# Eric-qi/RDO-PTQ

Measured on AMD Instinct MI355X. Metric: calibration images/sec (Cheng2020 W8A8 task-oriented RDO-PTQ, image-iterations over all units), higher is better.
Workload: dtype f32

## Files before the change

rdo-ptq_amd/csrc/fused_tail.hip:

```cpp
#include "rdo_common.h"
#include "gather_body.h"

namespace {

using namespace rdo::gq;
typedef unsigned short u16;
typedef unsigned u32x2 __attribute__((ext_vector_type(2)));

inline unsigned loss_grid(long blocks) {
    const long cap = rdo::tuning(rdo::T_TAIL_GRID);
    return (unsigned)(blocks < 1 ? 1 : (blocks > cap ? cap : blocks));
}

using rdo::grid_for;

__device__ __forceinline__ void block_loss_add(float acc, float scale, float* loss_out, int it, int32_t* pub) {
    if (pub && blockIdx.x == 0 && threadIdx.x == 0) *pub = it;
    acc = rdo::block_sum(acc);
    if (threadIdx.x == 0 && loss_out)
        atomicAdd(loss_out + (long)it * RDO_LOG_SLOTS + (blockIdx.x & (RDO_LOG_SLOTS - 1)), acc * scale);
}

__device__ __forceinline__ void load_h2_oct(const H2In& pl, long M, int C, const Oct& o, f32x4& a, f32x4& b) {
    const long pstride = M * C;
    const long e = ((long)(o.c0 >> 4) * M + o.m) * 16 + (o.c0 & 15);
    const u32x4 h = *reinterpret_cast<const u32x4*>(pl.p + e), l = *reinterpret_cast<const u32x4*>(pl.p + pstride + e);
    using rdo::h2_hi;
    using rdo::h2_lo;
    a = f32x4{(h2_lo(h[0]) + h2_lo(l[0])) * pl.inv, (h2_hi(h[0]) + h2_hi(l[0])) * pl.inv, (h2_lo(h[1]) + h2_lo(l[1])) * pl.inv,
              (h2_hi(h[1]) + h2_hi(l[1])) * pl.inv};
    b = f32x4{(h2_lo(h[2]) + h2_lo(l[2])) * pl.inv, (h2_hi(h[2]) + h2_hi(l[2])) * pl.inv, (h2_lo(h[3]) + h2_lo(l[3])) * pl.inv,
              (h2_hi(h[3]) + h2_hi(l[3])) * pl.inv};
}

__global__ __launch_bounds__(256) void gather_qdrop_h2_kernel(Gather g, const int32_t* iter_ptr, int32_t* iter_publish) {
    const int it = *iter_ptr;
// ... 79 lines not shown
            if (res) r[k] = ldq(res + e);
            acc += loss_act_quad(ldq(pre + e), ldq(yrow + e), has_r ? &r[k] : nullptr, act, slope, gs, o[k], g[k], d[k]);
        }
#pragma unroll
        for (int k = 0; k < 2; ++k) {
            if (out) stq(out + e0 + k * Q2, o[k]);
            if (gout) stq(gout + e0 + k * Q2, g[k]);
            if (dpre) stq(dpre + e0 + k * Q2, d[k]);
        }
        if (dpre_planes.p) store_h2_oct(dpre_planes, M, C, oc, d[0], d[1], bad);
    }
    if (dpre_planes.p) rdo::h2_report(bad, dpre_planes.ovf);
    block_loss_add(acc, inv_npix * coef, loss_out, it, iter_pub);
}

__device__ __forceinline__ float loss_gdn_quad(const f32x4& xv, const f32x4& nv, const f32x4& y, const f32x4* r, int inverse, float gs,
                                               f32x4& o, f32x4& g, f32x4& tv) {
    f32x4 rs;
#pragma unroll
    for (int k = 0; k < 4; ++k) {
        rs[k] = __frsqrt_rn(nv[k]);
        o[k] = xv[k] * (inverse ? __fsqrt_rn(nv[k]) : rs[k]);
    }
    if (r) o += *r;
    const f32x4 dd = o - y;
    g = dd * gs;
#pragma unroll
    for (int k = 0; k < 4; ++k)
        tv[k] = inverse ? (0.5f * g[k] * xv[k]) * rs[k] : (-0.5f * g[k] * xv[k]) * (rs[k] * rs[k] * rs[k]);
    return (dd[0] * dd[0] + dd[1] * dd[1]) + (dd[2] * dd[2] + dd[3] * dd[3]);
}

__global__ __launch_bounds__(256) void loss_gdn_bwd_kernel(const float* x, const float* nrm, const float* res, const float* tgt,
                                                           const int32_t* idx_table, const int32_t* iter_ptr, int B, long per_image,
                                                           float inv_npix, float coef, int inverse, float* out, float* gout, float* tbuf,
                                                           float* loss_out, int32_t* iter_pub) {
    const int it = *iter_ptr;
    const long quads = per_image / 4;
    const long total = (long)B * quads;
    const float gs = coef * 2.f * inv_npix;
    float acc = 0.f;
    for (long q = (long)blockIdx.x * blockDim.x + threadIdx.x; q < total; q += (long)gridDim.x * blockDim.x) {
        const int b = (int)(q / quads);
        const long off = (q - (long)b * quads) * 4;
        const long e = (long)b * per_image + off;
        f32x4 r, o, g, tv;
        if (res) r = ldq(res + e);
// ... 31 lines not shown
            if (res) r = ldq(res + e);
            acc += loss_gdn_quad(ldq(x + e), ldq(nrm + e), ldq(yrow + e), res ? &r : nullptr, inverse, gs, o[k], g[k], tv[k]);
        }
#pragma unroll
        for (int k = 0; k < 2; ++k) {
            if (out) stq(out + e0 + k * Q2, o[k]);
            stq(gout + e0 + k * Q2, g[k]);
            if (tbuf) stq(tbuf + e0 + k * Q2, tv[k]);
        }
        store_h2_oct(t_planes, M, C, oc, tv[0], tv[1], bad);
    }
    rdo::h2_report(bad, t_planes.ovf);
    block_loss_add(acc, inv_npix * coef, loss_out, it, iter_pub);
}

__device__ __forceinline__ f32x4 gdn_dx_quad(const f32x4& gv, const f32x4& xv, const f32x4& nv, const f32x4& av, int inverse) {
    f32x4 o;
#pragma unroll
    for (int k = 0; k < 4; ++k) {
        const float f = inverse ? __fsqrt_rn(nv[k]) : __frsqrt_rn(nv[k]);
        o[k] = gv[k] * f + 2.f * xv[k] * av[k];
    }
    return o;
}

__global__ __launch_bounds__(256) void gdn_bwd_dx_kernel(const float* g, const float* x, const float* nrm, const float* acc, long n4,
                                                         int inverse, float* dx) {
    for (long q = (long)blockIdx.x * blockDim.x + threadIdx.x; q < n4; q += (long)gridDim.x * blockDim.x) {
        const long e = q * 4;
        stq(dx + e, gdn_dx_quad(ldq(g + e), ldq(x + e), ldq(nrm + e), ldq(acc + e), inverse));
    }
}

__global__ __launch_bounds__(256) void gdn_bwd_dx_pix_kernel(const float* g, const float* x, const float* nrm, const float* acc, long M,
                                                             int C, int inverse, float* dx, H2Out dx_planes) {
    int bad = 0;
    const int ngroups = (C + 31) / 32;
    const long nvb = ((M + 63) / 64) * ngroups;
    for (long vb = blockIdx.x; vb < nvb; vb += gridDim.x) {
        Oct oc;
// ... 269 lines not shown
```

rdo-ptq_amd/csrc/linear_h2.hip:

```cpp
#include <cstdlib>

#include "rdo_common.h"

namespace {

typedef float f32x4 __attribute__((ext_vector_type(4)));
typedef _Float16 f16x8 __attribute__((ext_vector_type(8)));
typedef _Float16 f16x4 __attribute__((ext_vector_type(4)));
typedef unsigned u32x4 __attribute__((ext_vector_type(4)));

constexpr int BM = 64;
constexpr int KB = 192;
constexpr int NC = 192;
constexpr int SLICES = KB / 16;
constexpr int PLANE = SLICES * BM * 32;
constexpr int LDS_BYTES = 2 * PLANE + 2 * BM * 4;

struct LinArgs {
    const float* x;
    const unsigned short* wp;
    const float* bias;
    float* out;
    int M, K, N;
    float inv_wscale;
    int square;
#ifdef RDO_DIAG
    int diag;
#endif
    int epi;
    float* pre;
    const float* aux;
};

__device__ __forceinline__ float pow2f(int e) { return __builtin_bit_cast(float, (unsigned)(e + 127) << 23); }

template <int EPI, bool PART = false>
__global__ __launch_bounds__(256, 3) void linear_h2_kernel(LinArgs a) {
    extern __shared__ __attribute__((aligned(16))) char smem[];
    float* scl = reinterpret_cast<float*>(smem + 2 * PLANE);
    const int tid = threadIdx.x, lane = tid & 63, wave = tid >> 6;
    const int l16 = lane & 15, kg = lane >> 4;
    const int nkb = PART ? (a.K + KB - 1) / KB : a.K / KB, nchunks = PART ? (a.N + NC - 1) / NC : a.N / NC, nblk = a.N / 16, ksteps = a.K / 32;
    const int kvalid4 = PART ? (a.K < KB ? a.K : KB) >> 2 : KB / 4;
    const int nks = PART ? (ksteps < KB / 32 ? ksteps : KB / 32) : KB / 32;
    const bool wave_live = !PART || a.N >= NC || wave * 48 < a.N;
    int wg_tile, wg_chunk;
    {
        const int ntiles = a.M / BM;
        const int id = blockIdx.x, xcd = id & 7, slot = id >> 3;
// ... 27 lines not shown
#pragma unroll
                for (int k = 0; k < 3; ++k)
                    if (l16 + 16 * k >= kvalid4) v[pass][k] = f32x4{0.f, 0.f, 0.f, 0.f};
        }
        if (a.square) {
#pragma unroll
            for (int pass = 0; pass < BM / 16; ++pass)
#pragma unroll
                for (int k = 0; k < 3; ++k) v[pass][k] *= v[pass][k];
        }
#pragma unroll
        for (int pass = 0; pass < BM / 16; ++pass) {
            const int r = pass * 16 + row_in_pass;
            float amax = 0.f;
#pragma unroll
            for (int k = 0; k < 3; ++k)
                amax = fmaxf(amax, fmaxf(fmaxf(fabsf(v[pass][k][0]), fabsf(v[pass][k][1])), fmaxf(fabsf(v[pass][k][2]), fabsf(v[pass][k][3]))));
            amax = fmaxf(amax, __shfl_xor(amax, 8, 16));
            amax = fmaxf(amax, __shfl_xor(amax, 4, 16));
            amax = fmaxf(amax, __shfl_xor(amax, 2, 16));
            amax = fmaxf(amax, __shfl_xor(amax, 1, 16));
            const int e = (int)((__builtin_bit_cast(unsigned, amax) >> 23) & 0xFF) - 127;
            const bool plain = e < -100 || e > 100;
            const float s = plain ? 1.f : pow2f(7 - e);
            if (l16 == 0) scl[(kb & 1) * BM + r] = plain ? 1.f : pow2f(e - 7);
#pragma unroll
            for (int k = 0; k < 3; ++k) {
                const int c4 = l16 + 16 * k;
                const f32x4 xs = v[pass][k] * s;
                const f16x4 hi = __builtin_convertvector(xs, f16x4);
                const f16x4 lo = __builtin_convertvector(xs - __builtin_convertvector(hi, f32x4), f16x4);
                char* dst = smem + (c4 >> 2) * (BM * 32) + r * 32 + (c4 & 3) * 8;
                *reinterpret_cast<f16x4*>(dst) = hi;
                *reinterpret_cast<f16x4*>(dst + PLANE) = lo;
            }
        }
    };

    const u32x4* wbase = reinterpret_cast<const u32x4*>(a.wp) + lane;
    auto load_w = [&](f16x8 (&fw)[2][3], int ks, int chunk) {
        const long b0 = wave_live ? (long)chunk * (NC / 16) + wave * 3 : 0;
#pragma unroll
        for (int p = 0; p < 2; ++p)
#pragma unroll
            for (int i = 0; i < 3; ++i)
                fw[p][i] = __builtin_bit_cast(f16x8, wbase[(((long)p * ksteps + ks) * nblk + b0 + i) * 64]);
    };
    const int fx_lane = (kg >> 1) * (BM * 32) + l16 * 32 + (kg & 1) * 16;
    auto read_x = [&](f16x8 (&fx)[2][4], int ksl) {
// ... 124 lines not shown
        for (int pass = 0; pass < 2; ++pass)
#pragma unroll
            for (int k = 0; k < 3; ++k) asm volatile("" : "+v"(v[pass][k]));
    };
    auto stash = [&](int p) {
        char* buf = smem + (p & 1) * BUF;
#pragma unroll
        for (int pass = 0; pass < 2; ++pass) {
            const int r = pass * 32 + row_in_pass;
            if (a.square) {
#pragma unroll
                for (int k = 0; k < 3; ++k) v[pass][k] *= v[pass][k];
            }
            float amax = 0.f;
#pragma unroll
            for (int k = 0; k < 3; ++k)
                amax = fmaxf(amax, fmaxf(fmaxf(fabsf(v[pass][k][0]), fabsf(v[pass][k][1])), fmaxf(fabsf(v[pass][k][2]), fabsf(v[pass][k][3]))));
            amax = fmaxf(amax, __shfl_xor(amax, 8, 16));
            amax = fmaxf(amax, __shfl_xor(amax, 4, 16));
            amax = fmaxf(amax, __shfl_xor(amax, 2, 16));
            amax = fmaxf(amax, __shfl_xor(amax, 1, 16));
            const int e = (int)((__builtin_bit_cast(unsigned, amax) >> 23) & 0xFF) - 127;
            const bool plain = e < -100 || e > 100;
            const float sc = plain ? 1.f : pow2f(7 - e);
            if (l16 == 0) scl[(p & 3) * BM + r] = plain ? 1.f : pow2f(e - 7);
#pragma unroll
            for (int k = 0; k < 3; ++k) {
                const int c4 = l16 + 16 * k;
                const f32x4 xs = v[pass][k] * sc;
                const f16x4 hi = __builtin_convertvector(xs, f16x4);
                const f16x4 lo = __builtin_convertvector(xs - __builtin_convertvector(hi, f32x4), f16x4);
                char* dst = buf + (c4 >> 2) * (BM * 32) + r * 32 + (c4 & 3) * 8;
                *reinterpret_cast<f16x4*>(dst) = hi;
                *reinterpret_cast<f16x4*>(dst + PLANE) = lo;
            }
        }
    };

    int tl = grp;
    fetch(first + tl, 0);
    if (tid < NCW) bsm[tid] = a.bias ? a.bias[chunk * NCW + tid] : 0.f;
    f16x8 fw[2][KS][NT];
    {
        const u32x4* wbase = reinterpret_cast<const u32x4*>(a.wp) + lane;
        const long b0 = (long)chunk * (NCW / 16) + cg * NT;
        u32x4 raw[2][KS][NT];
#pragma unroll
        for (int p = 0; p < 2; ++p)
#pragma unroll
// ... 239 lines not shown
```

rdo-ptq_amd/hipops/_lib.py:

```python
import ctypes as C
import os

_HERE = os.path.dirname(os.path.abspath(__file__))
LIB_PATH = os.path.join(os.path.dirname(_HERE), "lib", "librdoptq_hip.so")

EPI_NONE, EPI_LRELU, EPI_LRELU_BWD, EPI_GDN, EPI_IGDN, EPI_RELU, EPI_RELU_BWD, EPI_GELU, EPI_GELU_BWD = range(9)
LOG_SLOTS = 32


class ConvDesc(C.Structure):
    _fields_ = [(n, C.c_int32) for n in ("B", "H", "W", "Cin", "Ho", "Wo", "Cout", "KH", "KW", "stride", "pad", "epilogue",
                                         "square_input", "add_residual")]


class AdaDesc(C.Structure):
    _fields_ = [("numel", C.c_int64), ("rows", C.c_int32), ("n_levels", C.c_int32), ("reparam", C.c_int32),
                ("reparam_bound", C.c_float), ("reparam_pedestal", C.c_float), ("KH", C.c_int32), ("KW", C.c_int32),
                ("Cin", C.c_int32)]


class AdaStepItem(C.Structure):
    _fields_ = [("d", AdaDesc), ("w", C.c_void_p), ("delta", C.c_void_p), ("zp", C.c_void_p), ("slabs", C.c_void_p),
                ("nsplit", C.c_int32), ("alpha", C.c_void_p), ("adam_m", C.c_void_p), ("adam_v", C.c_void_p), ("wq", C.c_void_p),
                ("wd", C.c_void_p), ("wq_planes", C.c_void_p), ("wd_planes", C.c_void_p), ("dalpha", C.c_void_p),
# ... 132 lines not shown
    "rdo_pixel_shuffle_h2": (C.c_int, [P, C.c_int32, C.c_int32, C.c_int32, C.c_int32, P, P, C.c_float, P]),
    "rdo_pixel_unshuffle2": (C.c_int, [P, C.c_int32, C.c_int32, C.c_int32, C.c_int32, P, P, C.c_float, P]),
    "rdo_plan_create": (P, []),
    "rdo_plan_destroy": (None, [P]),
    "rdo_plan_begin_record": (C.c_int, [P]),
    "rdo_plan_end_record": (C.c_int, [P]),
    "rdo_plan_suspend_record": (C.c_int, [C.c_int]),
    "rdo_plan_num_ops": (C.c_int, [P]),
    "rdo_plan_run": (C.c_int, [P, C.c_int, C.c_int, P]),
    "rdo_plan_prepare": (C.c_int, [P, C.c_int]),
    "rdo_plan_run_then": (C.c_int, [P, P, C.c_int, P]),
    "rdo_plan_op_info": (C.c_int, [P, C.c_int, C.POINTER(C.c_char_p), C.POINTER(C.c_double), C.POINTER(C.c_double)]),
    "rdo_plan_profile": (C.c_int, [P, C.POINTER(C.c_float), P]),
}
EXPORTS = tuple(_SIGS)

_lib = None


def lib():
    global _lib
    if _lib is None:
        if not os.path.exists(LIB_PATH):
            raise RuntimeError(f"{LIB_PATH} not found: build it with `python __graft_entry__.py` or "
                               f"`make -C rdo-ptq_amd/csrc` (no CPU fallback exists)")
        import torch
        h = C.CDLL(LIB_PATH)
        for name, (res, args) in _SIGS.items():
            fn = getattr(h, name)
            fn.restype, fn.argtypes = res, args
        _lib = h
    return _lib


def check(rc, what=""):
    if rc != 0:
        raise RuntimeError(f"librdoptq_hip {what} failed ({rc}): {lib().rdo_last_error().decode()}")
```

rdo-ptq_amd/hipops/ops.py:

```python
import ctypes as C
import math
import threading

import torch

from . import _lib as L


class H2:
    __slots__ = ("t", "scale", "flag")

    def __init__(self, t, scale, flag=None):
        self.t, self.scale = t, float(scale)
        self.flag = flag
        m, e = math.frexp(self.scale)
        if not (self.scale > 0 and m == 0.5):
            raise ValueError(f"H2 scale must be a positive power of two, got {scale}")

    @property
    def device(self):
        return self.t.device


def _ptr(t):
# ... 1247 lines not shown

def loss_gdn_bwd(x, norm, residual, tgt_cache, idx_table, iter_ptr, coef, inverse, loss_log, grad_out, t=None, t_planes=None, out=None):
    B, per_image = x.shape[0], x[0].numel()
    _bind_out(t_planes)
    L.check(L.lib().rdo_loss_gdn_bwd(_ptr(x), _ptr(norm), _ptr(residual), _ptr(tgt_cache), _ptr(idx_table), _ptr(iter_ptr), B, per_image,
                                     x.shape[-1], coef, int(inverse), _ptr(out), _ptr(grad_out), _ptr(t), _ptr(t_planes), _oscale(t_planes),
                                     _ptr(loss_log), _stream()), "rdo_loss_gdn_bwd")


def gdn_bwd_dx_h2(g, x, norm, acc, inverse, dx=None, dx_planes=None):
    _bind_out(dx_planes)
    L.check(L.lib().rdo_gdn_bwd_dx_h2(_ptr(g), _ptr(x), _ptr(norm), _ptr(acc), g.numel(), g.shape[-1], int(inverse), _ptr(dx),
                                      _ptr(dx_planes), _oscale(dx_planes), _stream()), "rdo_gdn_bwd_dx_h2")


def pixel_shuffle_h2(x, out=None, out_planes=None):
    B, H, W, CC = x.shape
    _bind_out(out_planes)
    L.check(L.lib().rdo_pixel_shuffle_h2(_ptr(x), B, H, W, CC // 4, _ptr(out), _ptr(out_planes), _oscale(out_planes), _stream()),
            "rdo_pixel_shuffle_h2")


def pixel_unshuffle2(x, out=None, out_planes=None):
    B, Hr, Wr, Cc = x.shape
    if out is None and out_planes is None:
        out = torch.empty((B, Hr // 2, Wr // 2, 4 * Cc), device=x.device, dtype=torch.float32)
    _bind_out(out_planes)
    L.check(L.lib().rdo_pixel_unshuffle2(_ptr(x), B, Hr // 2, Wr // 2, Cc, _ptr(out), _ptr(out_planes), _oscale(out_planes), _stream()),
            "rdo_pixel_unshuffle2")
    return out
# ... 20 lines not shown
```

rdo-ptq_amd/quantization/engine.py:

```python
import math
import os
from collections import OrderedDict

import torch

from hipops import _lib as L
from hipops import ops
from hipops.plan import Plan

from . import dp
from .quant_layer import QuantModule
from .quantizer import AdaRoundQuantizer, from_rows, to_rows

UNIT_KINDS = ("layer", "rb", "rbws", "rbu", "rstb")


class DpStallError(RuntimeError):
    """The captured data-parallel loop stopped making progress (`UnitEngine._hb_wait`): a collective inside the graph hangs."""


class IdxStream:
    _spec = None

    @classmethod
# ... 203 lines not shown
        self.task_p = float(task_p)
        self.weight, self.input_prob, self.seed = float(weight), float(input_prob), int(seed) & 0xFFFFFFFF
        self.include_act = include_act_func
        self.use_graph = use_graph
        self.batch_offset = int(batch_offset)
        self.dp_overlap = None if dp_overlap is None else bool(dp_overlap)
        if os.environ.get("RDO_USE_H2") is not None:
            use_h2 = os.environ["RDO_USE_H2"] != "0"
        self.use_h2 = bool(use_h2)
        self.P = {}
        self.batch_step = bool(batch_step)
        self.fuse_splitk = os.environ.get("RDO_FUSE_SPLITK", "1") != "0"
        self.fuse_h2_tail = os.environ.get("RDO_H2_TAIL", "1") != "0"
        self.fold_iter = os.environ.get("RDO_FOLD_ITER", "1") != "0"
        self.fold_gather = os.environ.get("RDO_GATHER_IN_STEP", "1") != "0"
        self._next_gather = None
        self.rd = rd
        if rd is not None:
            metric = rd.get("metric", "mse")
            if metric not in ("mse", "ms-ssim"):
                raise ValueError(f"loss_mode='rd': unknown metric {metric!r} ('mse' or 'ms-ssim')")
            if metric == "ms-ssim" and min(rd["cali"].shape[-2:]) <= 160:
                raise ValueError(f"loss_mode='rd' with metric 'ms-ssim' needs calibration crops with both sides above 160 pixels (five "
                                 f"scales of an 11-tap window); got {tuple(rd['cali'].shape[-2:])}")
            if not include_act_func:
                raise NotImplementedError("calibration engine: loss_mode='rd' substitutes the unit's module OUTPUT (after its fused "
                                          "activation); include_act_func=False optimises the pre-activation and cannot be combined with it")
            fuse_tail = use_h2 = False
            self.use_h2 = False
        self.fuse_tail = bool(fuse_tail)
# ... 117 lines not shown
            else:
                Ho, Wo = self._out_hw(op, H, W)
            t["y"] = self._buf(B, Ho, Wo, op.rows)
            t["dy"] = self._buf(B, Ho, Wo, op.rows)
            t["dpre"] = self._buf(B, Ho, Wo, op.rows)
        elif self.kind == "rb":
            C = o["conv1"].rows
            for n_ in ("h1", "pre2", "out", "dout", "dpre2", "dh1"):
                t[n_] = self._buf(B, H, W, C)
            if "skip" in o:
                t["sk"] = self._buf(B, H, W, C)
        elif self.kind == "rbws":
            c1 = o["conv1"]
            Ho, Wo = self._out_hw(c1, H, W)
            C = c1.rows
            for n_ in ("h1", "c2", "norm", "out", "dout", "t", "acc", "dc2", "dh1"):
                t[n_] = self._buf(B, Ho, Wo, C)
            if "skip" in o:
                t["sk"] = self._buf(B, Ho, Wo, C)
        elif self.kind == "rbu":
            sp = o["subpel_conv"]
            C4 = sp.rows
            r = int(self.mods["upscale"])
            C = C4 // (r * r)
            t["sp"] = self._buf(B, H, W, C4)
            t["h1"] = self._buf(B, H * r, W * r, C)
            t["up"] = self._buf(B, H, W, C4)
            t["ups"] = self._buf(B, H * r, W * r, C)
            for n_ in ("c", "norm", "out", "dout", "t", "acc", "dc", "dh1"):
                t[n_] = self._buf(B, H * r, W * r, C)
            t["dsp"] = self._buf(B, H, W, C4)
            t["dup"] = self._buf(B, H, W, C4)
            self.r = r
        self.t = t
        for op in self.ops.values():
            op.slabs = None

    def _slabs(self, op, x_shape):
        ns = ops.wgrad_nsplit(tuple(x_shape), op.w4, op.stride, op.pad)
        op.slabs = self._buf(ns, *op.w4)
        return op.slabs

    lin_conv = os.environ.get("RDO_CONV1X1_LIN_H2", "1") != "0"

    def _lin_conv_ok(self, op, x):
        if not (self.lin_conv and not self._probing and op.qm.kind == "conv" and op.K == 1 and op.stride == 1 and op.pad == 0 and op.tconv is None):
            return False
        C = x.shape[-1]
        rows = math.prod(x.shape[:-1])
        return rows >= self.LIN_GDN_MIN_ROWS and ops.linear_h2_supported(rows, C, op.w4[0])

# ... 339 lines not shown
            if side_first:
                self._shuffle(t["up"], r, t["ups"])
            self._conv(cv, h1, c)
            if not side_first:
                self._conv(side, x, t["up"])
                self._shuffle(t["up"], r, t["ups"])
            res = t["ups"]
        else:
            self._conv(first, x, h1, epilogue=L.EPI_LRELU)
            if side is not None and side_first:
                self._conv(side, x.f32, t["sk"])
            self._conv(cv, h1, c)
            if side is not None and not side_first:
                self._conv(side, x.f32, t["sk"])
            res = x if side is None else t["sk"]
        if self.fused:
            self._gdn_pool(g, c, t["norm"])
            self._tail_gdn(c, t["norm"], res, rbu, t["dout"], tt)
        else:
            self._conv(g, c, t["out"], epilogue=L.EPI_IGDN if rbu else L.EPI_GDN, aux=c, residual=res, pre=t["norm"], square=True)
            self._loss(t["out"], t["dout"])
        if rbu:
            dup = self._act("dup")
            self._unshuffle(t["dout"], r, dup)
            self._wgrad(side, x, dup)
        elif side is not None:
            self._wgrad(side, x.f32, t["dout"])
        if not self.fused:
            ops.gdn_bwd_t(t["dout"], c, t["norm"], rbu, tt.f32)
        self._gdn_acc(g, tt, t["acc"])
        if dc.planes is not None or c.numel() % 4 == 0:
            ops.gdn_bwd_dx_h2(t["dout"], c, t["norm"], t["acc"], rbu, dx=dc.f32, dx_planes=dc.planes)
        else:
            ops.gdn_bwd_dx(t["dout"], c, t["norm"], t["acc"], rbu, dc.f32)
        self._wgrad(g, c, tt.f32, square=True)
        self._wgrad(cv, h1, dc)
        dh1 = self._act("dh1")
        self._dgrad(cv, dc, dh1, epilogue=L.EPI_LRELU_BWD, aux=h1)
        if rbu:
            dsp = self._act("dsp")
            self._unshuffle(dh1, r, dsp)
            self._split_point()
            self._wgrad(first, x, dsp)
        else:
            self._split_point()
            self._wgrad(first, x, dh1)

    def _probe_amax(self, names):
        saved = ops.set_tuning("conv_x6", 0)
# ... 11 lines not shown
            if op.tc_phase is not None:
                op.expand_phase()

    def _probe_scales(self):
        plan = self._plan_h2()
        if plan is None:
            return
        names = [self.PLANES_AS.get(n, n) for n, f in self._forms(plan, widest=True).items() if f & PLANES]
        amax = self._probe_amax(names)
        self._set_weights(soft=False)
        try:
            amax = torch.maximum(amax, self._probe_amax(names))
        finally:
            self._set_weights(soft=True)
        self._clear_probe()
        if self.world > 1:
            a = amax.to(self.dev)
            a = torch.where(torch.isfinite(a), a, torch.full_like(a, float("inf")))
            torch.distributed.all_reduce(a, op=torch.distributed.ReduceOp.MAX, group=self.group)
            amax = a.cpu()
        if not torch.isfinite(amax).all():
            raise RuntimeError("calibration engine: non-finite activations in the probe iteration")
        if bool((amax <= 0).any()):
            import logging
            logging.getLogger("rdo_ptq.engine").warning(
                "unit with an all-zero tensor in both probe iterations (%s): no fp16 plane scale can be derived, running it on fp32 activations",
                [n for n, a in zip(names, amax) if float(a) <= 0])
            self.use_h2 = False
            return
        self._amax = {n: float(a) for n, a in zip(names, amax)}
# ... 568 lines not shown
```

Baseline: 20440.

## Fuse GDN forward, loss, backward-t and dx into one MFMA kernel

Adds a single kernel that squares the conv output, runs the gamma GEMM on fp16 hi/lo planes with MFMA, applies the GDN/IGDN epilogue with the reconstruction loss, computes t, runs the transposed gamma GEMM and writes dx (optionally as fp16 planes). It replaces the separate pool, tail, gdn_acc and bwd_dx launches and removes the norm/acc intermediate tensors from global memory. The engine uses it when C=192 and the row count is a multiple of 64, and drops the now-unused buffers after probing. The trade-off is a larger, more complex kernel with high register/LDS use and only two blocks per CU, limited to one channel width.

Result: faster. 21240, median of 6 (+3.9%).

```diff
diff --git a/include/rdo_ptq_gdn.h b/include/rdo_ptq_gdn.h
--- /dev/null
+++ b/include/rdo_ptq_gdn.h
@@ -0,0 +1,18 @@
+#ifndef RDO_PTQ_GDN_H
+#define RDO_PTQ_GDN_H
+#include "rdo_ptq_hip.h"
+
+#ifdef __cplusplus
+extern "C" {
+#endif
+
+int rdo_gdn_fwd_bwd_supported(int64_t M, int32_t C);
+int rdo_gdn_fwd_bwd(const float* c, const void* fwd_planes, const void* bwd_planes, float wscale, const float* beta, const float* residual,
+                    const float* tgt_cache, const int32_t* idx_table, const int32_t* iter_ptr, int32_t B, int64_t per_image, int32_t C,
+                    float coef, int32_t inverse, float* out, float* grad_out, float* t, float* dx, void* dx_planes, float dx_scale,
+                    float* loss_out, void* stream);
+
+#ifdef __cplusplus
+}
+#endif
+#endif
diff --git a/rdo-ptq_amd/csrc/fused_tail.hip b/rdo-ptq_amd/csrc/fused_tail.hip
--- a/rdo-ptq_amd/csrc/fused_tail.hip
+++ b/rdo-ptq_amd/csrc/fused_tail.hip
@@ -1,5 +1,6 @@
 #include "rdo_common.h"
 #include "gather_body.h"
+#include "gdn_device.h"
 
 namespace {
 
@@ -13,13 +14,9 @@
 }
 
 using rdo::grid_for;
-
-__device__ __forceinline__ void block_loss_add(float acc, float scale, float* loss_out, int it, int32_t* pub) {
-    if (pub && blockIdx.x == 0 && threadIdx.x == 0) *pub = it;
-    acc = rdo::block_sum(acc);
-    if (threadIdx.x == 0 && loss_out)
-        atomicAdd(loss_out + (long)it * RDO_LOG_SLOTS + (blockIdx.x & (RDO_LOG_SLOTS - 1)), acc * scale);
-}
+using rdo::gdn::block_loss_add;
+using rdo::gdn::loss_gdn_quad;
+using rdo::gdn::gdn_dx_quad;
 
 __device__ __forceinline__ void load_h2_oct(const H2In& pl, long M, int C, const Oct& o, f32x4& a, f32x4& b) {
     const long pstride = M * C;
@@ -129,23 +126,6 @@
     block_loss_add(acc, inv_npix * coef, loss_out, it, iter_pub);
 }
 
-__device__ __forceinline__ float loss_gdn_quad(const f32x4& xv, const f32x4& nv, const f32x4& y, const f32x4* r, int inverse, float gs,
-                                               f32x4& o, f32x4& g, f32x4& tv) {
-    f32x4 rs;
-#pragma unroll
-    for (int k = 0; k < 4; ++k) {
-        rs[k] = __frsqrt_rn(nv[k]);
-        o[k] = xv[k] * (inverse ? __fsqrt_rn(nv[k]) : rs[k]);
-    }
-    if (r) o += *r;
-    const f32x4 dd = o - y;
-    g = dd * gs;
-#pragma unroll
-    for (int k = 0; k < 4; ++k)
-        tv[k] = inverse ? (0.5f * g[k] * xv[k]) * rs[k] : (-0.5f * g[k] * xv[k]) * (rs[k] * rs[k] * rs[k]);
-    return (dd[0] * dd[0] + dd[1] * dd[1]) + (dd[2] * dd[2] + dd[3] * dd[3]);
-}
-
 __global__ __launch_bounds__(256) void loss_gdn_bwd_kernel(const float* x, const float* nrm, const float* res, const float* tgt,
                                                            const int32_t* idx_table, const int32_t* iter_ptr, int B, long per_image,
                                                            float inv_npix, float coef, int inverse, float* out, float* gout, float* tbuf,
@@ -207,16 +187,6 @@
     block_loss_add(acc, inv_npix * coef, loss_out, it, iter_pub);
 }
 
-__device__ __forceinline__ f32x4 gdn_dx_quad(const f32x4& gv, const f32x4& xv, const f32x4& nv, const f32x4& av, int inverse) {
-    f32x4 o;
-#pragma unroll
-    for (int k = 0; k < 4; ++k) {
-        const float f = inverse ? __fsqrt_rn(nv[k]) : __frsqrt_rn(nv[k]);
-        o[k] = gv[k] * f + 2.f * xv[k] * av[k];
-    }
-    return o;
-}
-
 __global__ __launch_bounds__(256) void gdn_bwd_dx_kernel(const float* g, const float* x, const float* nrm, const float* acc, long n4,
                                                          int inverse, float* dx) {
     for (long q = (long)blockIdx.x * blockDim.x + threadIdx.x; q < n4; q += (long)gridDim.x * blockDim.x) {
diff --git a/rdo-ptq_amd/csrc/gdn_device.h b/rdo-ptq_amd/csrc/gdn_device.h
--- /dev/null
+++ b/rdo-ptq_amd/csrc/gdn_device.h
@@ -0,0 +1,87 @@
+#pragma once
+#include "rdo_common.h"
+
+namespace rdo {
+namespace gdn {
+
+typedef float f32x4 __attribute__((ext_vector_type(4)));
+typedef _Float16 f16x4 __attribute__((ext_vector_type(4)));
+
+__device__ __forceinline__ float pow2f(int e) { return __builtin_bit_cast(float, (unsigned)(e + 127) << 23); }
+
+__device__ __forceinline__ float amax_quad(const f32x4& v) { return fmaxf(fmaxf(fabsf(v[0]), fabsf(v[1])), fmaxf(fabsf(v[2]), fabsf(v[3]))); }
+
+__device__ __forceinline__ void token_scale(float amax, float& sc, float& inv) {
+    const int e = (int)((__builtin_bit_cast(unsigned, amax) >> 23) & 0xFF) - 127;
+    const bool plain = e < -100 || e > 100;
+    sc = plain ? 1.f : pow2f(7 - e);
+    inv = plain ? 1.f : pow2f(e - 7);
+}
+
+__device__ __forceinline__ void split_quad_store(const f32x4& v, float sc, char* dst, int plane) {
+    const f32x4 xs = v * sc;
+    const f16x4 hi = __builtin_convertvector(xs, f16x4);
+    const f16x4 lo = __builtin_convertvector(xs - __builtin_convertvector(hi, f32x4), f16x4);
+    *reinterpret_cast<f16x4*>(dst) = hi;
+    *reinterpret_cast<f16x4*>(dst + plane) = lo;
+}
+
+__device__ __forceinline__ void block_loss_add(float acc, float scale, float* loss_out, int it, int32_t* pub) {
+    if (pub && blockIdx.x == 0 && threadIdx.x == 0) *pub = it;
+    acc = rdo::block_sum(acc);
+    if (threadIdx.x == 0 && loss_out)
+        atomicAdd(loss_out + (long)it * RDO_LOG_SLOTS + (blockIdx.x & (RDO_LOG_SLOTS - 1)), acc * scale);
+}
+
+__device__ __forceinline__ void block_loss_add8(float acc, float scale, float* loss_out, int it, int32_t* pub, float* red) {
+    if (pub && blockIdx.x == 0 && threadIdx.x == 0) *pub = it;
+    for (int o = 32; o > 0; o >>= 1) acc += __shfl_down(acc, o, 64);
+    if ((threadIdx.x & 63) == 0) red[threadIdx.x >> 6] = acc;
+    __syncthreads();
+    if (threadIdx.x == 0 && loss_out) {
+        float v = red[0];
+#pragma unroll
+        for (int w = 1; w < 8; ++w) v += red[w];
+        atomicAdd(loss_out + (long)it * RDO_LOG_SLOTS + (blockIdx.x & (RDO_LOG_SLOTS - 1)), v * scale);
+    }
+}
+
+__device__ __forceinline__ float loss_gdn_quad(const f32x4& xv, const f32x4& nv, const f32x4& y, const f32x4* r, int inverse, float gs,
+                                               f32x4& o, f32x4& g, f32x4& tv) {
+    f32x4 rs;
+#pragma unroll
+    for (int k = 0; k < 4; ++k) {
+        rs[k] = __frsqrt_rn(nv[k]);
+        o[k] = xv[k] * (inverse ? __fsqrt_rn(nv[k]) : rs[k]);
+    }
+    if (r) o += *r;
+    const f32x4 dd = o - y;
+    g = dd * gs;
+#pragma unroll
+    for (int k = 0; k < 4; ++k)
+        tv[k] = inverse ? (0.5f * g[k] * xv[k]) * rs[k] : (-0.5f * g[k] * xv[k]) * (rs[k] * rs[k] * rs[k]);
+    return (dd[0] * dd[0] + dd[1] * dd[1]) + (dd[2] * dd[2] + dd[3] * dd[3]);
+}
+
+__device__ __forceinline__ void gdn_dx_pre(const f32x4& gv, const f32x4& xv, const f32x4& nv, int inverse, f32x4& p, f32x4& q) {
+#pragma unroll
+    for (int k = 0; k < 4; ++k) {
+        const float f = inverse ? __fsqrt_rn(nv[k]) : __frsqrt_rn(nv[k]);
+        p[k] = gv[k] * f;
+        q[k] = 2.f * xv[k];
+    }
+}
+__device__ __forceinline__ f32x4 gdn_dx_fin(const f32x4& p, const f32x4& q, const f32x4& av) {
+    f32x4 o;
+#pragma unroll
+    for (int k = 0; k < 4; ++k) o[k] = p[k] + q[k] * av[k];
+    return o;
+}
+__device__ __forceinline__ f32x4 gdn_dx_quad(const f32x4& gv, const f32x4& xv, const f32x4& nv, const f32x4& av, int inverse) {
+    f32x4 p, q;
+    gdn_dx_pre(gv, xv, nv, inverse, p, q);
+    return gdn_dx_fin(p, q, av);
+}
+
+}
+}
diff --git a/rdo-ptq_amd/csrc/gdn_fused.hip b/rdo-ptq_amd/csrc/gdn_fused.hip
--- /dev/null
+++ b/rdo-ptq_amd/csrc/gdn_fused.hip
@@ -0,0 +1,277 @@
+#include "rdo_common.h"
+#include "gather_body.h"
+#include "gdn_device.h"
+#include "../../include/rdo_ptq_gdn.h"
+
+namespace {
+
+using namespace rdo::gdn;
+using rdo::gq::H2Out;
+typedef _Float16 f16x8 __attribute__((ext_vector_type(8)));
+typedef unsigned u32x4 __attribute__((ext_vector_type(4)));
+typedef unsigned u32x2 __attribute__((ext_vector_type(2)));
+typedef unsigned short u16;
+
+constexpr int BM = 64;
+constexpr int CH = 192;
+constexpr int KS = CH / 32;
+constexpr int NBLK = CH / 16;
+constexpr int PLANE = (CH / 16) * BM * 32;
+constexpr int LDS_BYTES = 2 * PLANE + BM * 4 + 4 * BM * 4 + 8 * 4;
+
+struct GdnArgs {
+    const float* c;
+    const u16* wf;
+    const u16* wb;
+    const float* beta;
+    const float* res;
+    const float* tgt;
+    const int32_t* idx;
+    const int32_t* iter;
+    int32_t* pub;
+    int B, ntiles, inverse;
+    long per_image, M;
+    float inv_wscale, inv_npix, coef;
+    float* out;
+    float* gout;
+    float* t;
+    float* dx;
+    H2Out dxp;
+    float* loss_out;
+};
+
+__device__ __forceinline__ const f32x4& ldq(const float* p) { return *reinterpret_cast<const f32x4*>(p); }
+__device__ __forceinline__ void stq(float* p, const f32x4& v) { *reinterpret_cast<f32x4*>(p) = v; }
+
+template <bool INV, bool RES>
+__global__ __launch_bounds__(512, 2) void gdn_fwd_bwd_kernel(GdnArgs a) {
+    extern __shared__ __attribute__((aligned(16))) char smem[];
+    float* scl = reinterpret_cast<float*>(smem + 2 * PLANE);
+    float* wmax = scl + BM;
+    float* wsum = wmax + 4 * BM;
+    const int tid = threadIdx.x, lane = tid & 63, wave = __builtin_amdgcn_readfirstlane(tid >> 6);
+    const int cg = wave & 3, th = wave >> 2;
+    const int l16 = lane & 15, kg = lane >> 4;
+    const int it = *a.iter;
+    const float gs = a.coef * 2.f * a.inv_npix;
+    const long ppi = a.per_image / CH;
+    const int ch0 = 48 * cg + 4 * kg;
+    const unsigned lane_e = (unsigned)((32 * th + l16) * CH + ch0);
+    float lsum = 0.f;
+    int bad = 0;
+
+    const auto rs_f = __builtin_amdgcn_make_buffer_rsrc(const_cast<u16*>(a.wf), 0, 2 * CH * CH * 2, 0x00020000);
+    const auto rs_b = __builtin_amdgcn_make_buffer_rsrc(const_cast<u16*>(a.wb), 0, 2 * CH * CH * 2, 0x00020000);
+    auto load_w = [&](f16x8 (&fw)[2][3], const decltype(rs_f)& planes, int ks) {
+#pragma unroll
+        for (int p = 0; p < 2; ++p)
+#pragma unroll
+            for (int i = 0; i < 3; ++i)
+                fw[p][i] = __builtin_bit_cast(f16x8, __builtin_amdgcn_raw_buffer_load_b128(planes, (unsigned)lane * 16u,
+                                                                                           ((p * KS + ks) * NBLK + cg * 3 + i) * 1024, 0));
+    };
+    const int fx_lane = (kg >> 1) * (BM * 32) + (32 * th + l16) * 32 + (kg & 1) * 16;
+    auto gemm = [&](const decltype(rs_f)& planes, f32x4 (&acc)[3][2]) {
+        f16x8 fw[2][2][3];
+        load_w(fw[0], planes, 0);
+        __syncthreads();
+#pragma unroll
+        for (int i = 0; i < 3; ++i)
+#pragma unroll
+            for (int j = 0; j < 2; ++j) acc[i][j] = f32x4{0.f, 0.f, 0.f, 0.f};
+#pragma unroll
+        for (int ks = 0; ks < KS; ++ks) {
+            if (ks + 1 < KS) load_w(fw[(ks + 1) & 1], planes, ks + 1);
+            __builtin_amdgcn_sched_barrier(0);
+            f16x8 fx[2][2];
+#pragma unroll
+            for (int p = 0; p < 2; ++p)
+#pragma unroll
+                for (int j = 0; j < 2; ++j)
+                    fx[p][j] = *reinterpret_cast<const f16x8*>(smem + p * PLANE + (2 * ks) * (BM * 32) + j * (16 * 32) + fx_lane);
+            const int c = ks & 1;
+#pragma unroll
+            for (int i = 0; i < 3; ++i)
+#pragma unroll
+                for (int j = 0; j < 2; ++j) acc[i][j] = __builtin_amdgcn_mfma_f32_16x16x32_f16(fw[c][1][i], fx[0][j], acc[i][j], 0, 0, 0);
+#pragma unroll
+            for (int i = 0; i < 3; ++i)
+#pragma unroll
+                for (int j = 0; j < 2; ++j) acc[i][j] = __builtin_amdgcn_mfma_f32_16x16x32_f16(fw[c][0][i], fx[1][j], acc[i][j], 0, 0, 0);
+#pragma unroll
+            for (int i = 0; i < 3; ++i)
+#pragma unroll
+                for (int j = 0; j < 2; ++j) acc[i][j] = __builtin_amdgcn_mfma_f32_16x16x32_f16(fw[c][0][i], fx[0][j], acc[i][j], 0, 0, 0);
+            __builtin_amdgcn_sched_barrier(0);
+        }
+    };
+
+    f32x4 bq[3];
+#pragma unroll
+    for (int i = 0; i < 3; ++i) bq[i] = ldq(a.beta + ch0 + 16 * i);
+
+    for (int tile = blockIdx.x; tile < a.ntiles; tile += gridDim.x) {
+        const long m0 = (long)tile * BM;
+        {
+            const int row_in_pass = tid >> 4;
+            f32x4 v[2][3];
+#pragma unroll
+            for (int pass = 0; pass < 2; ++pass) {
+                const float* src = a.c + (m0 + pass * 32) * CH;
+#pragma unroll
+                for (int k = 0; k < 3; ++k) v[pass][k] = ldq(src + (unsigned)(row_in_pass * CH + 4 * l16) + 64 * k);
+            }
+#pragma unroll
+            for (int pass = 0; pass < 2; ++pass) {
+                const int r = pass * 32 + row_in_pass;
+                float amax = 0.f;
+#pragma unroll
+                for (int k = 0; k < 3; ++k) {
+                    v[pass][k] *= v[pass][k];
+                    amax = fmaxf(amax, amax_quad(v[pass][k]));
+                }
+                amax = fmaxf(amax, __shfl_xor(amax, 8, 16));
+                amax = fmaxf(amax, __shfl_xor(amax, 4, 16));
+                amax = fmaxf(amax, __shfl_xor(amax, 2, 16));
+                amax = fmaxf(amax, __shfl_xor(amax, 1, 16));
+                float sc, inv;
+                token_scale(amax, sc, inv);
+                if (l16 == 0) scl[r] = inv;
+#pragma unroll
+                for (int k = 0; k < 3; ++k) {
+                    const int c4 = l16 + 16 * k;
+                    split_quad_store(v[pass][k], sc, smem + (c4 >> 2) * (BM * 32) + r * 32 + (c4 & 3) * 8, PLANE);
+                }
+            }
+        }
+        f32x4 acc[3][2];
+        gemm(rs_f, acc);
+        f32x4 p[3][2], q[3][2];
+#pragma unroll
+        for (int j = 0; j < 2; ++j) {
+            const int tok = 32 * th + 16 * j + l16;
+            const long m = m0 + tok;
+            const int b = (int)(m / ppi);
+            const long g0 = (m0 + 16 * j) * CH;
+            const float* yrow = a.tgt + ((long)a.idx[(long)it * a.B + b] - b) * a.per_image + m * CH + ch0;
+            const float f = scl[tok] * a.inv_wscale;
+            f32x4 xv[3], yv[3], rv[3];
+#pragma unroll
+            for (int i = 0; i < 3; ++i) {
+                xv[i] = ldq(a.c + g0 + lane_e + 16 * i);
+                yv[i] = ldq(yrow + 16 * i);
+                if (RES) rv[i] = ldq(a.res + g0 + lane_e + 16 * i);
+            }
+            float tmax = 0.f;
+#pragma unroll
+            for (int i = 0; i < 3; ++i) {
+                f32x4 n = acc[i][j] * f;
+                n += bq[i];
+                f32x4 o, g, tv;
+                lsum += loss_gdn_quad(xv[i], n, yv[i], RES ? &rv[i] : nullptr, INV ? 1 : 0, gs, o, g, tv);
+                if (a.out) stq(a.out + g0 + lane_e + 16 * i, o);
+                if (a.gout) stq(a.gout + g0 + lane_e + 16 * i, g);
+                stq(a.t + g0 + lane_e + 16 * i, tv);
+                f32x4 nd = n;
+                if (INV) asm volatile("" : "+v"(nd));
+                gdn_dx_pre(g, xv[i], nd, INV ? 1 : 0, p[i][j], q[i][j]);
+                acc[i][j] = tv;
+                tmax = fmaxf(tmax, amax_quad(tv));
+            }
+            tmax = fmaxf(tmax, __shfl_xor(tmax, 16, 64));
+            tmax = fmaxf(tmax, __shfl_xor(tmax, 32, 64));
+            if (kg == 0) wmax[cg * BM + tok] = tmax;
+        }
+        __syncthreads();
+        float inv_t[2];
+#pragma unroll
+        for (int j = 0; j < 2; ++j) {
+            const int tok = 32 * th + 16 * j + l16;
+            const float amax = fmaxf(fmaxf(wmax[tok], wmax[BM + tok]), fmaxf(wmax[2 * BM + tok], wmax[3 * BM + tok]));
+            float sc;
+            token_scale(amax, sc, inv_t[j]);
+#pragma unroll
+            for (int i = 0; i < 3; ++i) split_quad_store(acc[i][j], sc, smem + (3 * cg + i) * (BM * 32) + tok * 32 + kg * 8, PLANE);
+        }
+        gemm(rs_b, acc);
+#pragma unroll
+        for (int j = 0; j < 2; ++j) {
+            const long g0 = (m0 + 16 * j) * CH;
+            const float f = inv_t[j] * a.inv_wscale;
+#pragma unroll
+            for (int i = 0; i < 3; ++i) {
+                const f32x4 av = acc[i][j] * f;
+                const f32x4 d = gdn_dx_fin(p[i][j], q[i][j], av);
+                if (a.dx) stq(a.dx + g0 + lane_e + 16 * i, d);
+                if (a.dxp.p) {
+                    const long e = ((long)(3 * cg + i) * a.M + m0 + 16 * j) * 16 + (unsigned)((32 * th + l16) * 16 + 4 * kg);
+                    unsigned h0, l0, h1, l1;
+                    rdo::h2_split_pk(d[0], d[1], a.dxp.s, h0, l0, bad);
+                    rdo::h2_split_pk(d[2], d[3], a.dxp.s, h1, l1, bad);
+                    *reinterpret_cast<u32x2*>(a.dxp.p + e) = u32x2{h0, h1};
+                    *reinterpret_cast<u32x2*>(a.dxp.p + a.M * CH + e) = u32x2{l0, l1};
+                }
+            }
+        }
+        __syncthreads();
+    }
+    if (a.dxp.p) rdo::h2_report(bad, a.dxp.ovf);
+    block_loss_add8(lsum, a.inv_npix * a.coef, a.loss_out, it, a.pub, wsum);
+}
+
+bool pow2(float s) {
+    if (!(s > 0.f) || s != s || s > 3.0e38f) return false;
+    int e;
+    return frexpf(s, &e) == 0.5f;
+}
+
+int cu_count() {
+    int dev = 0, n = 0;
+    if (hipGetDevice(&dev) != hipSuccess || hipDeviceGetAttribute(&n, hipDeviceAttributeMultiprocessorCount, dev) != hipSuccess || n < 1) n = 256;
+    return n;
+}
+
+}
+
+extern "C" int rdo_gdn_fwd_bwd_supported(int64_t M, int32_t C) {
+    return C == CH && M > 0 && M % BM == 0 && rdo_linear_h2_supported(M, C, C);
+}
+
+extern "C" int rdo_gdn_fwd_bwd(const float* c, const void* fwd_planes, const void* bwd_planes, float wscale, const float* beta,
+                               const float* residual, const float* tgt_cache, const int32_t* idx_table, const int32_t* iter_ptr, int32_t B,
+                               int64_t per_image, int32_t C, float coef, int32_t inverse, float* out, float* grad_out, float* t, float* dx,
+                               void* dx_planes, float dx_scale, float* loss_out, void* stream) {
+    RDO_REQUIRE(c && fwd_planes && bwd_planes && beta && tgt_cache && idx_table && iter_ptr && t, "rdo_gdn_fwd_bwd: null pointer");
+    RDO_REQUIRE(B > 0 && C > 0 && per_image > 0 && per_image % C == 0, "rdo_gdn_fwd_bwd: bad shape");
+    const int64_t M = (int64_t)B * (per_image / C);
+    RDO_REQUIRE(rdo_gdn_fwd_bwd_supported(M, C), "rdo_gdn_fwd_bwd: %ld tokens x %d channels is not supported (C = 192, tokens %% 64)", (long)M, C);
+    RDO_REQUIRE(pow2(wscale), "rdo_gdn_fwd_bwd: weight scale %g is not a power of two", (double)wscale);
+    RDO_REQUIRE(!dx_planes || dx_scale > 0.f, "rdo_gdn_fwd_bwd: dx_scale must be a positive power of two");
+    RDO_REQUIRE(((reinterpret_cast<uintptr_t>(c) | reinterpret_cast<uintptr_t>(fwd_planes) | reinterpret_cast<uintptr_t>(bwd_planes) |
+                  reinterpret_cast<uintptr_t>(beta) | reinterpret_cast<uintptr_t>(residual) | reinterpret_cast<uintptr_t>(tgt_cache) |
+                  reinterpret_cast<uintptr_t>(out) | reinterpret_cast<uintptr_t>(grad_out) | reinterpret_cast<uintptr_t>(t) |
+                  reinterpret_cast<uintptr_t>(dx) | reinterpret_cast<uintptr_t>(dx_planes)) & 15) == 0,
+                "rdo_gdn_fwd_bwd: pointers must be 16-byte aligned");
+    GdnArgs a;
+    a.c = c; a.wf = reinterpret_cast<const u16*>(fwd_planes); a.wb = reinterpret_cast<const u16*>(bwd_planes); a.beta = beta; a.res = residual;
+    a.tgt = tgt_cache; a.idx = idx_table; a.iter = iter_ptr; a.pub = rdo::take_iter_publish();
+    a.B = B; a.ntiles = (int)(M / BM); a.inverse = inverse ? 1 : 0; a.per_image = (long)per_image; a.M = (long)M;
+    a.inv_wscale = 1.0f / wscale; a.inv_npix = (float)(1.0 / (double)M); a.coef = coef;
+    a.out = out; a.gout = grad_out; a.t = t; a.dx = dx;
+    a.dxp = H2Out{reinterpret_cast<u16*>(dx_planes), dx_scale, rdo::h2_overflow_flag()};
+    a.loss_out = loss_out;
+    const double n = (double)M * C;
+    const double bytes = n * (12.0 + 4.0 * ((residual != nullptr) + (out != nullptr) + (grad_out != nullptr) + (dx != nullptr)) + (dx_planes ? 4.0 : 0.0)) +
+                         2.0 * 4.0 * C * C;
+    return rdo::dispatch(
+        [a](hipStream_t s) {
+            const int wgs = cu_count();
+            const dim3 grid((unsigned)(a.ntiles < wgs ? a.ntiles : wgs));
+            if (a.inverse && a.res) hipLaunchKernelGGL((gdn_fwd_bwd_kernel<true, true>), grid, dim3(512), LDS_BYTES, s, a);
+            else if (a.inverse) hipLaunchKernelGGL((gdn_fwd_bwd_kernel<true, false>), grid, dim3(512), LDS_BYTES, s, a);
+            else if (a.res) hipLaunchKernelGGL((gdn_fwd_bwd_kernel<false, true>), grid, dim3(512), LDS_BYTES, s, a);
+            else hipLaunchKernelGGL((gdn_fwd_bwd_kernel<false, false>), grid, dim3(512), LDS_BYTES, s, a);
+            return rdo::check_launch("gdn_fwd_bwd");
+        },
+        stream, "linear_h2_gdn", 2.0 * 2.0 * (double)M * C * C, bytes);
+}
diff --git a/rdo-ptq_amd/csrc/linear_h2.hip b/rdo-ptq_amd/csrc/linear_h2.hip
--- a/rdo-ptq_amd/csrc/linear_h2.hip
+++ b/rdo-ptq_amd/csrc/linear_h2.hip
@@ -1,8 +1,13 @@
 #include <cstdlib>
 
 #include "rdo_common.h"
+#include "gdn_device.h"
 
 namespace {
+
+using rdo::gdn::amax_quad;
+using rdo::gdn::token_scale;
+using rdo::gdn::split_quad_store;
 
 typedef float f32x4 __attribute__((ext_vector_type(4)));
 typedef _Float16 f16x8 __attribute__((ext_vector_type(8)));
@@ -31,8 +36,6 @@
     float* pre;
     const float* aux;
 };
-
-__device__ __forceinline__ float pow2f(int e) { return __builtin_bit_cast(float, (unsigned)(e + 127) << 23); }
 
 template <int EPI, bool PART = false>
 __global__ __launch_bounds__(256, 3) void linear_h2_kernel(LinArgs a) {
@@ -90,25 +93,18 @@
             const int r = pass * 16 + row_in_pass;
             float amax = 0.f;
 #pragma unroll
-            for (int k = 0; k < 3; ++k)
-                amax = fmaxf(amax, fmaxf(fmaxf(fabsf(v[pass][k][0]), fabsf(v[pass][k][1])), fmaxf(fabsf(v[pass][k][2]), fabsf(v[pass][k][3]))));
+            for (int k = 0; k < 3; ++k) amax = fmaxf(amax, amax_quad(v[pass][k]));
             amax = fmaxf(amax, __shfl_xor(amax, 8, 16));
             amax = fmaxf(amax, __shfl_xor(amax, 4, 16));
             amax = fmaxf(amax, __shfl_xor(amax, 2, 16));
             amax = fmaxf(amax, __shfl_xor(amax, 1, 16));
-            const int e = (int)((__builtin_bit_cast(unsigned, amax) >> 23) & 0xFF) - 127;
-            const bool plain = e < -100 || e > 100;
-            const float s = plain ? 1.f : pow2f(7 - e);
-            if (l16 == 0) scl[(kb & 1) * BM + r] = plain ? 1.f : pow2f(e - 7);
+            float s, inv;
+            token_scale(amax, s, inv);
+            if (l16 == 0) scl[(kb & 1) * BM + r] = inv;
 #pragma unroll
             for (int k = 0; k < 3; ++k) {
                 const int c4 = l16 + 16 * k;
-                const f32x4 xs = v[pass][k] * s;
-                const f16x4 hi = __builtin_convertvector(xs, f16x4);
-                const f16x4 lo = __builtin_convertvector(xs - __builtin_convertvector(hi, f32x4), f16x4);
-                char* dst = smem + (c4 >> 2) * (BM * 32) + r * 32 + (c4 & 3) * 8;
-                *reinterpret_cast<f16x4*>(dst) = hi;
-                *reinterpret_cast<f16x4*>(dst + PLANE) = lo;
+                split_quad_store(v[pass][k], s, smem + (c4 >> 2) * (BM * 32) + r * 32 + (c4 & 3) * 8, PLANE);
             }
         }
     };
@@ -263,25 +259,18 @@
             }
             float amax = 0.f;
 #pragma unroll
-            for (int k = 0; k < 3; ++k)
-                amax = fmaxf(amax, fmaxf(fmaxf(fabsf(v[pass][k][0]), fabsf(v[pass][k][1])), fmaxf(fabsf(v[pass][k][2]), fabsf(v[pass][k][3]))));
+            for (int k = 0; k < 3; ++k) amax = fmaxf(amax, amax_quad(v[pass][k]));
             amax = fmaxf(amax, __shfl_xor(amax, 8, 16));
             amax = fmaxf(amax, __shfl_xor(amax, 4, 16));
             amax = fmaxf(amax, __shfl_xor(amax, 2, 16));
             amax = fmaxf(amax, __shfl_xor(amax, 1, 16));
-            const int e = (int)((__builtin_bit_cast(unsigned, amax) >> 23) & 0xFF) - 127;
-            const bool plain = e < -100 || e > 100;
-            const float sc = plain ? 1.f : pow2f(7 - e);
-            if (l16 == 0) scl[(p & 3) * BM + r] = plain ? 1.f : pow2f(e - 7);
+            float sc, inv;
+            token_scale(amax, sc, inv);
+            if (l16 == 0) scl[(p & 3) * BM + r] = inv;
 #pragma unroll
             for (int k = 0; k < 3; ++k) {
                 const int c4 = l16 + 16 * k;
-                const f32x4 xs = v[pass][k] * sc;
-                const f16x4 hi = __builtin_convertvector(xs, f16x4);
-                const f16x4 lo = __builtin_convertvector(xs - __builtin_convertvector(hi, f32x4), f16x4);
-                char* dst = buf + (c4 >> 2) * (BM * 32) + r * 32 + (c4 & 3) * 8;
-                *reinterpret_cast<f16x4*>(dst) = hi;
-                *reinterpret_cast<f16x4*>(dst + PLANE) = lo;
+                split_quad_store(v[pass][k], sc, buf + (c4 >> 2) * (BM * 32) + r * 32 + (c4 & 3) * 8, PLANE);
             }
         }
     };
diff --git a/rdo-ptq_amd/hipops/_lib.py b/rdo-ptq_amd/hipops/_lib.py
--- a/rdo-ptq_amd/hipops/_lib.py
+++ b/rdo-ptq_amd/hipops/_lib.py
@@ -170,6 +170,11 @@
     "rdo_plan_profile": (C.c_int, [P, C.POINTER(C.c_float), P]),
 }
 EXPORTS = tuple(_SIGS)
+_SIGS_GDN = {
+    "rdo_gdn_fwd_bwd_supported": (C.c_int, [C.c_int64, C.c_int32]),
+    "rdo_gdn_fwd_bwd": (C.c_int, [P, P, P, C.c_float, P, P, P, P, P, C.c_int32, C.c_int64, C.c_int32, C.c_float, C.c_int32, P, P, P, P, P, C.c_float, P, P]),
+}
+EXPORTS_GDN = tuple(_SIGS_GDN)
 
 _lib = None
 
@@ -182,7 +187,7 @@
                                f"`make -C rdo-ptq_amd/csrc` (no CPU fallback exists)")
         import torch
         h = C.CDLL(LIB_PATH)
-        for name, (res, args) in _SIGS.items():
+        for name, (res, args) in list(_SIGS.items()) + list(_SIGS_GDN.items()):
             fn = getattr(h, name)
             fn.restype, fn.argtypes = res, args
         _lib = h
diff --git a/rdo-ptq_amd/hipops/ops.py b/rdo-ptq_amd/hipops/ops.py
--- a/rdo-ptq_amd/hipops/ops.py
+++ b/rdo-ptq_amd/hipops/ops.py
@@ -1285,6 +1285,22 @@
                                       _ptr(dx_planes), _oscale(dx_planes), _stream()), "rdo_gdn_bwd_dx_h2")
 
 
+def gdn_fwd_bwd_supported(rows, channels):
+    return bool(L.lib().rdo_gdn_fwd_bwd_supported(int(rows), int(channels)))
+
+
+def gdn_fwd_bwd(c, fwd_planes, bwd_planes, beta, residual, tgt_cache, idx_table, iter_ptr, coef, inverse, loss_log, t, grad_out=None, out=None,
+                dx=None, dx_planes=None):
+    if fwd_planes.scale != bwd_planes.scale:
+        raise ValueError("gdn_fwd_bwd: the planes of gamma' and of its transpose must share one scale")
+    B, per_image = c.shape[0], c[0].numel()
+    _bind_out(dx_planes)
+    L.check(L.lib().rdo_gdn_fwd_bwd(_ptr(c), _ptr(fwd_planes), _ptr(bwd_planes), float(fwd_planes.scale), _ptr(beta), _ptr(residual),
+                                    _ptr(tgt_cache), _ptr(idx_table), _ptr(iter_ptr), B, per_image, c.shape[-1], coef, int(inverse), _ptr(out),
+                                    _ptr(grad_out), _ptr(t), _ptr(dx), _ptr(dx_planes), _oscale(dx_planes), _ptr(loss_log), _stream()),
+            "rdo_gdn_fwd_bwd")
+
+
 def pixel_shuffle_h2(x, out=None, out_planes=None):
     B, H, W, CC = x.shape
     _bind_out(out_planes)
diff --git a/rdo-ptq_amd/quantization/engine.py b/rdo-ptq_amd/quantization/engine.py
--- a/rdo-ptq_amd/quantization/engine.py
+++ b/rdo-ptq_amd/quantization/engine.py
@@ -241,6 +241,7 @@
         self.fuse_h2_tail = os.environ.get("RDO_H2_TAIL", "1") != "0"
         self.fold_iter = os.environ.get("RDO_FOLD_ITER", "1") != "0"
         self.fold_gather = os.environ.get("RDO_GATHER_IN_STEP", "1") != "0"
+        self.gdn_fused = os.environ.get("RDO_GDN_FUSED", "1") != "0"
         self._next_gather = None
         self.rd = rd
         if rd is not None:
@@ -388,7 +389,7 @@
             c1 = o["conv1"]
             Ho, Wo = self._out_hw(c1, H, W)
             C = c1.rows
-            for n_ in ("h1", "c2", "norm", "out", "dout", "t", "acc", "dc2", "dh1"):
+            for n_ in ("h1", "c2", "out", "dout", "t", "dc2", "dh1"):
                 t[n_] = self._buf(B, Ho, Wo, C)
             if "skip" in o:
                 t["sk"] = self._buf(B, Ho, Wo, C)
@@ -401,7 +402,7 @@
             t["h1"] = self._buf(B, H * r, W * r, C)
             t["up"] = self._buf(B, H, W, C4)
             t["ups"] = self._buf(B, H * r, W * r, C)
-            for n_ in ("c", "norm", "out", "dout", "t", "acc", "dc", "dh1"):
+            for n_ in ("c", "out", "dout", "t", "dc", "dh1"):
                 t[n_] = self._buf(B, H * r, W * r, C)
             t["dsp"] = self._buf(B, H, W, C4)
             t["dup"] = self._buf(B, H, W, C4)
@@ -409,6 +410,13 @@
         self.t = t
         for op in self.ops.values():
             op.slabs = None
+
+    GDN_TMP = ("norm", "acc")
+
+    def _tmp(self, name, like):
+        if name not in self.t:
+            self.t[name] = self._buf(*like.shape)
+        return self.t[name]
 
     def _slabs(self, op, x_shape):
         ns = ops.wgrad_nsplit(tuple(x_shape), op.w4, op.stride, op.pad)
@@ -778,11 +786,17 @@
             if side is not None and not side_first:
                 self._conv(side, x.f32, t["sk"])
             res = x if side is None else t["sk"]
-        if self.fused:
-            self._gdn_pool(g, c, t["norm"])
+        one = (self.fused and self.gdn_fused and self._gdn_lin_ok(g, c) and tt.planes is None
+               and ops.gdn_fwd_bwd_supported(math.prod(c.shape[:-1]), c.shape[-1]))
+        if one:
+            self._task_is_rec = True
+            ops.gdn_fwd_bwd(c, g.lin_planes(True), g.lin_planes(False), g.beta, _f32(res), self.co, self.idx, self.it, 2.0, rbu, self.loss_log,
+                            tt.f32, grad_out=t["dout"] if (rbu or side is not None) else None, dx=dc.f32, dx_planes=dc.planes)
+        elif self.fused:
+            self._gdn_pool(g, c, self._tmp("norm", c))
             self._tail_gdn(c, t["norm"], res, rbu, t["dout"], tt)
         else:
-            self._conv(g, c, t["out"], epilogue=L.EPI_IGDN if rbu else L.EPI_GDN, aux=c, residual=res, pre=t["norm"], square=True)
+            self._conv(g, c, t["out"], epilogue=L.EPI_IGDN if rbu else L.EPI_GDN, aux=c, residual=res, pre=self._tmp("norm", c), square=True)
             self._loss(t["out"], t["dout"])
         if rbu:
             dup = self._act("dup")
@@ -792,11 +806,12 @@
             self._wgrad(side, x.f32, t["dout"])
         if not self.fused:
             ops.gdn_bwd_t(t["dout"], c, t["norm"], rbu, tt.f32)
-        self._gdn_acc(g, tt, t["acc"])
-        if dc.planes is not None or c.numel() % 4 == 0:
-            ops.gdn_bwd_dx_h2(t["dout"], c, t["norm"], t["acc"], rbu, dx=dc.f32, dx_planes=dc.planes)
-        else:
-            ops.gdn_bwd_dx(t["dout"], c, t["norm"], t["acc"], rbu, dc.f32)
+        if not one:
+            self._gdn_acc(g, tt, self._tmp("acc", c))
+            if dc.planes is not None or c.numel() % 4 == 0:
+                ops.gdn_bwd_dx_h2(t["dout"], c, t["norm"], t["acc"], rbu, dx=dc.f32, dx_planes=dc.planes)
+            else:
+                ops.gdn_bwd_dx(t["dout"], c, t["norm"], t["acc"], rbu, dc.f32)
         self._wgrad(g, c, tt.f32, square=True)
         self._wgrad(cv, h1, dc)
         dh1 = self._act("dh1")
@@ -838,6 +853,9 @@
         finally:
             self._set_weights(soft=True)
         self._clear_probe()
+        for n_ in self.GDN_TMP:
+            if self.kind in ("rbws", "rbu"):
+                self.t.pop(n_, None)
         if self.world > 1:
             a = amax.to(self.dev)
             a = torch.where(torch.isfinite(a), a, torch.full_like(a, float("inf")))
```
